# gudovskiy/contextflow

Measured on AMD Instinct MI355X. Metric: samples/s fwd+logdet (log p(x) (B,M)), CIFAR-10C conv flow, higher is better.
Workload: dtype f32

## Files before the change

contextflow_amd/csrc/cf_step.hip:

```cpp
#include "cf_step_common.h"
#include "cf_step_inv.h"
#include "cf_step_dispatch.h"

namespace {

struct StepArgs {
    const float* x;
    float* z;
    float* ldj;
    const float* ws;
    int B;
    int64_t xbs;
    bool sq;
    hipStream_t s;
    float* dbg = nullptr;
    const float* sb = nullptr;
    StepTape tp = kNoTape;
};

constexpr int kPrepBatch = 16;
struct StepPackBatch {
    const float *Wm[kPrepBatch], *t[kPrepBatch], *logs[kPrepBatch], *w1[kPrepBatch], *b1[kPrepBatch], *w2[kPrepBatch], *b2[kPrepBatch],
        *w3[kPrepBatch], *b3[kPrepBatch];
    float* ws[kPrepBatch];
// ... 138 lines not shown
constexpr int kChain = 4;
struct WsChain { const float* ws[kChain]; };

template <class G, int CTX, bool DUMP, bool DBG, bool LEVEL>
__device__ __forceinline__ void flow_step_phases(float* __restrict__ z, float* __restrict__ ldj_acc, const float* __restrict__ wsl, int B,
                                                 float* __restrict__ dbg_arg, const float* __restrict__ sb, StepTape tp, int tile, int wave_u = 0) {
    float* const dbg = DBG ? dbg_arg : nullptr;
    constexpr int C = G::C, HW = G::HW, PIX = G::PIX, HALF = G::HALF, HID = G::HID;
    constexpr int PTW = G::PTW, RT03 = G::RT03;
    constexpr int WPX = 32 * PTW;
    static_assert(!LEVEL || (CTX == 0 && !DUMP && !DBG && HW <= 32 * PTW), "level form: the evaluation step, log-det inside the wave");
    extern __shared__ __align__(16) float lds[];
    float* Y0 = lds;
    float* H1 = lds + HALF * PIX;

    const int tid_ = LEVEL ? wave_u * 64 + cf_lane_fresh() : (int)threadIdx.x;
    const int tid = tid_, wave = tid >> 6;
    int lane = tid & 63, li = lane & 31, lk = lane >> 5;
    const int ntiles = (B + G::SPW - 1) / G::SPW;
    const int64_t dbg_cols = (int64_t)ntiles * PIX;

    int pix[PTW], pin[PTW];
#pragma unroll
    for (int q = 0; q < PTW; ++q) {
        pix[q] = (wave * PTW + q) * 32 + li;
        pin[q] = pix[q] % HW;
    }
    {
        const int b0 = tile * G::SPW;
        int smp[PTW];
        bool live[PTW];
// ... 16 lines not shown
                const int idx = tile_row(r, lk);
                if (idx < HALF) Y0[idx * PIX + pix[q]] = acc0[0][q][r];
                y1[q][r] = (HALF <= 16) ? acc0[0][q][r + 8] : acc0[RT03 - 1][q][r];
            }
        if constexpr (LEVEL) {
#pragma unroll
            for (int q = 0; q < PTW; ++q)
#pragma unroll
                for (int r = 0; r < (HALF <= 16 ? 8 : 16); ++r) asm volatile("" : "+v"(y1[q][r]));
        }
        cf_wave_sync();
        if constexpr (!LEVEL) z_store<G>(z, Y0, b0, 0, B, wave, lane);
        if constexpr (DUMP) rows_store_t<G, HALF, HALF>(tp.y0, Y0, b0, B, wave, lane);
        if (dbg) {
            __syncthreads();
            for (int e = tid; e < HALF * PIX; e += 256) dbg[(int64_t)(e / PIX) * dbg_cols + (int64_t)tile * PIX + (e % PIX)] = Y0[e];
            __syncthreads();
        }

        f32x16 acc3[RT03][PTW];
        if constexpr (LEVEL) {
            conditioner_net<G, 0, false, 2>(acc3, lds, wsl, pix, pin, lane, tid, nullptr, 0, tile, nullptr, nullptr, tp, B);
            lane = cf_lane_fresh(); li = lane & 31; lk = lane >> 5;
#pragma unroll
            for (int q = 0; q < PTW; ++q) {
                pix[q] = (wave_u * PTW + q) * 32 + li;
                pin[q] = pix[q] % HW;
                smp[q] = b0 + pix[q] / HW;
                live[q] = smp[q] < B;
            }
#pragma unroll
            for (int rt = 0; rt < RT03; ++rt)
#pragma unroll
                for (int q = 0; q < PTW; ++q) acc3[rt][q] = bias_tile(wsl + G::OFF_B3 + rt * 32, lk);
            dense_phase<G, G::KS3, G::NG3, RT03>(acc3, ws_rsrc(wsl, G::WS_FLOATS), G::OFF_A3, H1, pix, lane);
        } else if constexpr (CTX == 0) {
            conditioner_net<G, 0, DUMP>(acc3, lds, wsl, pix, pin, lane, tid, dbg, dbg_cols, tile, nullptr, nullptr, tp, B);
        } else {
// ... 70 lines not shown
            if (tid < G::SPW && b0 + tid < B) {
                float sum = 0.f;
#pragma unroll
                for (int i = 0; i < TPS; ++i) {
                    const int t = tid * TPS + i;
                    sum += Y0[(t / PTW) * WPX + (t % PTW)];
                }
                ldj_acc[b0 + tid] += wsl[0] + sum;
            }
            __syncthreads();
        }
    }
}

template <class G, bool SQ, int CTX = 0, bool DUMP = false, bool DBG = false>
__global__ __launch_bounds__(256, G::MINW) void k_flow_step(const float* __restrict__ x, float* __restrict__ z,
                                                   float* __restrict__ ldj_acc, const float* __restrict__ ws, int B,
                                                   int64_t xbs, float* __restrict__ dbg_arg, int flags,
                                                   const float* __restrict__ sb, StepTape tp) {
    constexpr int XI = G::C * G::PTW / 8;
    extern __shared__ __align__(16) float lds[];
    float* H1 = lds + G::HALF * G::PIX;
    const int tid = threadIdx.x, lane = tid & 63, wave = tid >> 6;
    (void)flags;

    float4 xr[XI];
    const int tile = blockIdx.x;
    x_load<G, SQ>(xr, x, xbs, tile, B, wave, lane);
    x_to_lds<G, SQ>(xr, H1, wave, lane);
    flow_step_phases<G, CTX, DUMP, DBG, false>(z, ldj_acc, ws, B, dbg_arg, sb, tp, tile);
}
template <class G, bool SQ>
__global__ __launch_bounds__(256, G::MINW) void k_flow_step_level(const float* __restrict__ x, float* __restrict__ z,
                                                                  float* __restrict__ ldj_acc, const WsChain wc, int nsteps, int B, int64_t xbs) {
    constexpr int XI = G::C * G::PTW / 8;
    extern __shared__ __align__(16) float lds[];
    float* H1 = lds + G::HALF * G::PIX;
    const int tid = threadIdx.x, lane = tid & 63, wave = tid >> 6;
    const int tile = blockIdx.x, wave_u = __builtin_amdgcn_readfirstlane(wave);
    {
        float4 xr[XI];
        x_load<G, SQ>(xr, x, xbs, tile, B, wave, lane);
        x_to_lds<G, SQ>(xr, H1, wave, lane);
    }
#pragma unroll 1
// ... 763 lines not shown
    if (rc) return rc;
    int blocks = (G::WS_FLOATS + 255) / 256;
    if (blocks > 512) blocks = 512;
    k_step_pack<G><<<dim3(blocks, n), dim3(256), 0, s>>>(pb);
    return 0;
}

template <class G, bool SQ, int CTX, bool DUMP, bool DBG>
int launch_step_sq(const StepArgs& a) {
    constexpr size_t lds_bytes = (size_t)G::LDS_FLOATS * sizeof(float);
    if (lds_bytes > 64 * 1024) {
        static std::atomic<uint64_t> raised{0};
        if (int rc_ = cf_raise_dynamic_lds((const void*)k_flow_step<G, SQ, CTX, DUMP, DBG>, 160 * 1024, raised, __func__)) return rc_;
    }
    const int grid = (a.B + G::SPW - 1) / G::SPW;
    k_flow_step<G, SQ, CTX, DUMP, DBG><<<dim3(grid), dim3(256), lds_bytes, a.s>>>(a.x, a.z, a.ldj, a.ws, a.B, a.xbs, a.dbg, 0, a.sb, a.tp);
    return 0;
}
template <class G, int CTX = 0, bool DUMP = false, bool DBG = false>
int launch_step(const StepArgs& a) {
    if constexpr (CTX == 0) { if (a.sq) return launch_step_sq<G, true, CTX, DUMP, DBG>(a); }
    return launch_step_sq<G, false, CTX, DUMP, DBG>(a);
}

template <class G, bool SQ>
int launch_step_level_sq(const StepArgs& a, const WsChain& wc, int n) {
    constexpr size_t lds_bytes = (size_t)G::LDS_FLOATS * sizeof(float);
    if (lds_bytes > 64 * 1024) {
        static std::atomic<uint64_t> raised{0};
        if (int rc_ = cf_raise_dynamic_lds((const void*)k_flow_step_level<G, SQ>, 160 * 1024, raised, __func__)) return rc_;
    }
// ... 14 lines not shown
        case Kernel::None: return 0;
        case Kernel::Small_G8s: return step_macs_c2hw<G8s>();
        case Kernel::Small_G16s: return step_macs_c2hw<G16s>();
        case Kernel::Small_G8w: case Kernel::Inv_G8w: return step_macs_c2hw<G8w>();
        case Kernel::Small_G16w: case Kernel::Inv_G16w: return step_macs_c2hw<G16w>();
        case Kernel::Step_G8: case Kernel::Inv_G8: return step_macs_c2hw<G8>();
        case Kernel::Step_G16: case Kernel::Inv_G16: return step_macs_c2hw<G16>();
        case Kernel::Step_G32: case Kernel::Rs_G32: case Kernel::Inv_G32: return step_macs_c2hw<G32>();
        case Kernel::Step_G32v2: return step_macs_c2hw<G32v2>();
        case Kernel::Step_G32w: case Kernel::Inv_G32w: return step_macs_c2hw<G32w>();
        case Kernel::Step_G32w24: return step_macs_c2hw<G32w24>();
        case Kernel::Step_G64: case Kernel::Rs16_G64: case Kernel::Inv_G64: return step_macs_c2hw<G64>();
        case Kernel::Step_G64v2: return step_macs_c2hw<G64v2>();
        case Kernel::Step_G64w2: case Kernel::Inv_G64w2: return step_macs_c2hw<G64w2>();
        case Kernel::Step_G64w24: return step_macs_c2hw<G64w24>();
    }
    return 0;
}

static int launch_fwd(Kernel k, const StepArgs& a) {
    switch (k) {
        case Kernel::Small_G8s: return launch_step_small<G8s>(a);
        case Kernel::Small_G16s: return launch_step_small<G16s>(a);
        case Kernel::Small_G8w: return launch_step_small<G8w>(a);
        case Kernel::Small_G16w: return launch_step_small<G16w>(a);
        case Kernel::Step_G8: return launch_step<G8>(a);
        case Kernel::Step_G16: return launch_step<G16>(a);
        case Kernel::Step_G32: return launch_step<G32>(a);
        case Kernel::Step_G32v2: return launch_step<G32v2>(a);
        case Kernel::Step_G32w: return launch_step<G32w>(a);
        case Kernel::Step_G32w24: return launch_step<G32w24>(a);
        case Kernel::Step_G64: return launch_step<G64>(a);
        case Kernel::Step_G64v2: return launch_step<G64v2>(a);
        case Kernel::Step_G64w2: return launch_step<G64w2>(a);
        case Kernel::Step_G64w24: return launch_step<G64w24>(a);
        case Kernel::Rs_G32: return launch_step_rs<G32, 2>(a);
        case Kernel::Rs16_G64: return launch_step_rs16<G64>(a);
        default: return not_built(__func__, k);
    }
}
static int launch_fwd_dumps(Kernel k, const StepArgs& a) {
    switch (k) {
        case Kernel::Small_G8s: return launch_step_small<G8s, true>(a);
        case Kernel::Small_G16s: return launch_step_small<G16s, true>(a);
        case Kernel::Step_G8: return launch_step<G8, 0, false, true>(a);
        case Kernel::Step_G16: return launch_step<G16, 0, false, true>(a);
        case Kernel::Step_G32: return launch_step<G32, 0, false, true>(a);
        case Kernel::Step_G64: return launch_step<G64, 0, false, true>(a);
        default: return not_built(__func__, k);
    }
// ... 82 lines not shown

template <class G>
static int lane_table_copy(int* out, int cap) {
    static const LaneTab<G> tab = make_lane_tab<G>();
    constexpr int n = (int)(sizeof(LaneEntry<G>) / sizeof(int));
    static_assert(sizeof(tab) == 256 * n * sizeof(int), "an entry is n ints, no padding");
    const int* src = reinterpret_cast<const int*>(&tab);
    for (int i = 0; out && i < cap && i < 256 * n; ++i) out[i] = src[i];
    return n;
}
constexpr int kDebugVariants = 8;
constexpr Kernel kDebugKernel[4][kDebugVariants] = {
    {Kernel::Step_G8, Kernel::None, Kernel::None, Kernel::Small_G8s, Kernel::Small_G8w, Kernel::None, Kernel::None, Kernel::None},
    {Kernel::Step_G16, Kernel::None, Kernel::None, Kernel::Small_G16s, Kernel::Small_G16w, Kernel::None, Kernel::None, Kernel::None},
    {Kernel::Step_G32, Kernel::None, Kernel::Step_G32v2, Kernel::None, Kernel::Step_G32w, Kernel::None, Kernel::Step_G32w24, Kernel::None},
    {Kernel::Step_G64, Kernel::None, Kernel::Step_G64v2, Kernel::None, Kernel::None, Kernel::Step_G64w2, Kernel::Step_G64w24, Kernel::None},
};

extern "C" {

int cf_flow_step_supported(int C, int H, int W, int kh, int kw) {
    return (kh == 3 && kw == 3 && shape_id(C, H, W) >= 0) ? 1 : 0;
}

int64_t cf_flow_step_ws_bytes(int C, int H, int W) {
    switch (shape_id(C, H, W)) {
        case 0: return (int64_t)G8::WS_FLOATS * 4;
        case 1: return (int64_t)G16::WS_FLOATS * 4;
        case 2: return (int64_t)G32::WS_FLOATS * 4;
        case 3: return (int64_t)G64::WS_FLOATS * 4;
    }
// ... 129 lines not shown
    if (B == 0) return 0;
    CF_REQUIRE(x && z && ldj_acc && ws && B >= 0 && x_bstride >= (int64_t)C * H * W);
    CF_REQUIRE((reinterpret_cast<uintptr_t>(x) & 15) == 0 && (reinterpret_cast<uintptr_t>(z) & 15) == 0 && x_bstride % 4 == 0);
    const int sid = shape_id(C, H, W), variant = (flags >> 16) & 15;
    const Kernel k = (sid >= 0 && variant < kDebugVariants) ? kDebugKernel[sid][variant] : Kernel::None;
    if (k == Kernel::None) {
        cf_set_error("cf_flow_step_fwd: shape (%d,%d,%d) variant %d unsupported", C, H, W, variant);
        return CF_ERR_UNSUPPORTED;
    }
    StepArgs a{x, z, ldj_acc, (const float*)ws, B, x_bstride, in_squeeze != 0, cf_s(stream)};
    a.dbg = dbg;
    if (int rc = dbg ? launch_fwd_dumps(k, a) : launch_fwd(k, a)) return rc;
    CF_LAUNCH_CHECK();
    return 0;
}
int cf_lane_table_debug(int C, int H, int W, int* out, int cap) {
    switch (shape_id(C, H, W)) {
        case 1: static_assert(kLaneTabW22<G16w>, "16x16, C = 16: F(2x2) table"); return lane_table_copy<G16w>(out, cap);
        case 2: static_assert(kLaneTabW24<G32w24>, "8x8: F(2x4) table"); return lane_table_copy<G32w24>(out, cap);    }
    return 0;
}
int cf_flow_step_chain_max_batch(int C, int H, int W) { return chain_max_batch(shape_id(C, H, W)); }

int cf_flow_step_fwd_chain(const float* x, float* z, float* ldj_acc, const void* const* ws, int n, int B, int C, int H, int W,
                           int64_t x_bstride, int in_squeeze, cf_stream_t stream) {
    if (B == 0 || n == 0) return 0;
    CF_REQUIRE(x && z && ldj_acc && ws && n >= 1 && n <= kChain && B > 0 && x_bstride >= (int64_t)C * H * W);
    CF_REQUIRE((reinterpret_cast<uintptr_t>(x) & 15) == 0 && (reinterpret_cast<uintptr_t>(z) & 15) == 0 && x_bstride % 4 == 0);
    const Kernel k = select(Pass::Chain, shape_id(C, H, W), B);
    if (k == Kernel::None) {
// ... 8 lines not shown
}

int cf_flow_step_level_min_batch(int C, int H, int W) { return level_min_batch(shape_id(C, H, W)); }

int cf_flow_step_fwd_level(const float* x, float* z, float* ldj_acc, const void* const* ws, int n, int B, int C, int H, int W,
                           int64_t x_bstride, int in_squeeze, int form, cf_stream_t stream) {
    if (B == 0 || n == 0) return 0;
    CF_REQUIRE(x && z && x != z && ldj_acc && ws && n >= 1 && n <= kChain && B > 0 && x_bstride >= (int64_t)C * H * W && (form == 0 || form == 1));
    CF_REQUIRE((reinterpret_cast<uintptr_t>(x) & 15) == 0 && (reinterpret_cast<uintptr_t>(z) & 15) == 0 && x_bstride % 4 == 0);
    const int sid = shape_id(C, H, W), minb = level_min_batch(sid);
    if (sid < 0) return unsupported_shape(__func__, C, H, W);
    if (minb == 0 || (form == 0 && B < minb)) {
        cf_set_error("cf_flow_step_fwd_level: shape (%d,%d,%d) at a batch of %d is not a level case", C, H, W, B);
        return CF_ERR_UNSUPPORTED;
    }
    const Kernel k = select(Pass::Eval, sid, form == 1 && B < minb ? minb : B);
    WsChain wc{};
    for (int i = 0; i < n; ++i) { CF_REQUIRE(ws[i]); wc.ws[i] = (const float*)ws[i]; }
    if (int rc = launch_fwd_level(k, StepArgs{x, z, ldj_acc, nullptr, B, x_bstride, in_squeeze != 0, cf_s(stream)}, wc, n)) return rc;
    CF_LAUNCH_CHECK();
    return 0;
}

int cf_flow_step_fwd(const float* x, float* z, float* ldj_acc, const void* ws, int B, int C, int H, int W,
                     int64_t x_bstride, int in_squeeze, cf_stream_t stream) {
    if (B == 0) return 0;
    CF_REQUIRE(x && z && ldj_acc && ws && B >= 0 && x_bstride >= (int64_t)C * H * W);
    CF_REQUIRE((reinterpret_cast<uintptr_t>(x) & 15) == 0 && (reinterpret_cast<uintptr_t>(z) & 15) == 0 && x_bstride % 4 == 0);
    const Kernel k = select(Pass::Eval, shape_id(C, H, W), B);
    if (k == Kernel::None) return unsupported_shape(__func__, C, H, W);
    if (int rc = launch_fwd(k, StepArgs{x, z, ldj_acc, (const float*)ws, B, x_bstride, in_squeeze != 0, cf_s(stream)})) return rc;
// ... 68 lines not shown
```

contextflow_amd/csrc/cf_step_common.h:

```cpp
#pragma once
#include <type_traits>
#include "cf_common.h"
#include <math.h>

namespace {


typedef float f32x16 __attribute__((ext_vector_type(16)));

constexpr int kWaves = 4;

template <int C_, int H_, int W_, int SPW_, int PIPE_ = 1, int ABL_ = 0, int PATCH_ = 0>
struct Geo {
    static constexpr int C = C_, H = H_, W = W_, SPW = SPW_, PIPE = PIPE_, ABL = ABL_, PATCH = PATCH_;
    static constexpr int HW = H * W;
    static constexpr int PIX = SPW * HW;
    static constexpr int HALF = C / 2;
    static constexpr int HID = 2 * C;
    static constexpr int NPT = PIX / 32;
    static constexpr int PTW = NPT / kWaves;
    static constexpr int HP = HALF <= 16 ? 16 : 32;
    static constexpr int R03 = 2 * HP;
    static constexpr int RT03 = R03 / 32;
    static constexpr int RT1 = (HID + 31) / 32;
    static constexpr int R1 = RT1 * 32;
    static constexpr int KS0 = C / 2, KS1 = HALF / 2, KS3 = HID / 2;
    static constexpr int NG0 = (KS0 + 3) / 4, NG1 = (KS1 + 3) / 4, NG3 = (KS3 + 3) / 4;
    static constexpr int NCG = HID / 8;
    static constexpr int NG2 = 9 * NCG;
    static constexpr int OFF_B0 = 4, OFF_B1 = OFF_B0 + R03, OFF_B2 = OFF_B1 + R1, OFF_B3 = OFF_B2 + R1;
    static constexpr int OFF_A0 = OFF_B3 + R03;
    static constexpr int OFF_A1 = OFF_A0 + NG0 * RT03 * 256;
    static constexpr int OFF_A2 = OFF_A1 + NG1 * RT1 * 256;
    static constexpr int OFF_A3 = OFF_A2 + NG2 * RT1 * 256;
    static constexpr bool SMALL = (H == 16 && W == 16 && SPW == 1 && C <= 16);
// ... 14 lines not shown
    static constexpr int OFF_RA0 = OFF_RB3 + C, OFF_RA1 = OFF_RA0 + (C / 16) * (C / 16) * 256;
    static constexpr int OFF_RA2 = OFF_RA1 + (HID / 16) * (HALF / 16) * 256, OFF_RA3 = OFF_RA2 + (HID / 16) * 9 * (HID / 16) * 256;
    static constexpr int R16_END = OFF_RA3 + (C / 16) * (HID / 16) * 256;
    static constexpr int WS_END0 = RS16 ? R16_END : OFF_AW + 16 * HID * HID;
    static constexpr bool HAS_W24 = (H == 4 && W == 4) || (H == 8 && W == 8);
    static constexpr int OFF_AW24 = WS_END0;
    static constexpr int WS_FLOATS = OFF_AW24 + (HAS_W24 ? 24 * HID * HID : 0);
    static constexpr int PP = 2 * W + 2 * H + 4;
    static constexpr int RS = PATCH ? ((PIX + SPW * PP + 1 + 3) & ~3) : PIX;
#ifndef CF_WINO_LDSW
#define CF_WINO_LDSW 1
#endif
    static constexpr int LDS_W = (CF_WINO_LDSW && PIPE_ == 3 && HID == 16 && H == 16 && W == 16 && SPW == 1) ? 16 * HID * HID : 0;
    static constexpr int LDS_FLOATS = (HALF + HID) * RS + LDS_W;
    static constexpr int MINW = (160 * 1024) / (LDS_FLOATS * 4) >= 4 ? 4 : ((160 * 1024) / (LDS_FLOATS * 4) >= 2 ? 2 : 1);
    static_assert(PIX % 128 == 0 && PTW >= 1, "workgroup must own a multiple of 128 pixels");
    static_assert(!W24 || (H == 4 && W == 4 && SPW == 8) || (H == 8 && W == 8 && SPW == 4),
                  "F(2x4, 3x3): 4x4 images, 8 samples = one column tile of 16 output tiles; 8x8 images, 4 samples = two column tiles");
    static_assert(HID % 8 == 0 && C % 4 == 0, "channel counts must fill whole k-steps");
    static_assert((HW & (HW - 1)) == 0 && (W & (W - 1)) == 0, "power-of-two images");
};

template <class G> constexpr bool kLaneTabW24 = G::W24 && G::H == 8;
template <class G> constexpr bool kLaneTabW22 = G::PIPE == 3 && G::SMALL && G::C == 16;

template <class G> __host__ __device__ constexpr int chan_of_row(int p) {
    return ((p % G::HP) < G::HALF) ? (p / G::HP) * G::HALF + (p % G::HP) : -1;
}

template <class G> __host__ __device__ constexpr int chan_of_row16(int p) {
    return (2 * (p >> 2) + (p & 1) < G::HALF) ? ((p & 2) ? G::HALF : 0) + 2 * (p >> 2) + (p & 1) : -1;
}

// ... 586 lines not shown
#pragma unroll
            for (int i = 0; i < 2; ++i) {
                float* dst = kLaneTabW22<G> ? H1 + (rt0 + rt) * 16 * PIX + i * W + dsto
                                            : H1 + ((rt0 + rt) * 16 + 4 * lg) * PIX + smp[ct] * HW + (2 * ty[ct] + i) * W + 2 * tx[ct];
                const float bb[4] = {b.x, b.y, b.z, b.w};
#pragma unroll
                for (int r = 0; r < 4; ++r)
                    *reinterpret_cast<float2*>(dst + r * PIX) =
                        make_float2(cf_relu(Y[ct][i][0][rt][r] + bb[r]), cf_relu(Y[ct][i][1][rt][r] + bb[r]));
            }
    }
    if constexpr (RSPLIT > 1) __syncthreads();
    else cf_wave_sync();
}

template <class G> __host__ __device__ constexpr int w24_row(int s, int y, int kq) {
    return 128 * (s >> 1) + 32 * ((y ^ (kq >> 1)) & 1) + 8 * (y >> 1) + 4 * (s & 1);
}
template <class G> __host__ __device__ constexpr int w24_col(int x, int kq) {
    return 64 * ((x >> 1) & 1) + 2 * (((x >> 2) ^ (x >> 1)) & 1) + ((x ^ kq) & 1);
}
template <class G> __host__ __device__ constexpr int w24_pix(int s, int y, int x, int kq) {
    if constexpr (G::H == 4) return 8 * (4 * y + ((x + y + kq) & 3)) + s;
    else return w24_row<G>(s, y, kq) + w24_col<G>(x, kq);
}

constexpr int cf_reflect(int v, int n) { return v < 0 ? -v : (v >= n ? 2 * (n - 1) - v : v); }
template <class G> struct alignas(16) W24Lane {
    int row[4];
    int col[6];
    int dst;
    int pad;
    int pw[G::PTW][4];
};
template <class G> __host__ __device__ constexpr W24Lane<G> w24_lane(int wave, int lane) {
    static_assert(kLaneTabW24<G>, "tabulated for the 8x8 level");
    constexpr int W = G::W, H = G::H, HW = G::HW, PIX = G::PIX, HALF = G::HALF, NCT = PIX / 128, TPS = HW / 8, TXN = W / 4;
    W24Lane<G> e{};
// ... 23 lines not shown
    const int l15 = lane & 15, lg = lane >> 4, li = lane & 31;
    const int tg = wave * 16 + l15, ti = tg % TPS;
    const int smp = tg / TPS, ty = ti / (W / 2), tx = ti % (W / 2);
    for (int a = 0; a < 4; ++a) {
        const int yy = cf_reflect(2 * ty - 1 + a, H), xx = cf_reflect(2 * tx - 1 + a, W);
        e.row[a] = 4 * (HALF * PIX + lg * PIX + wino_pix<G>(smp * HW, yy, 0));
        e.col[a] = 4 * ((((xx ^ lg) & 1) * (W / 2)) + (xx >> 1));
    }
    for (int q = 0; q < 2; ++q) {
        const int pix = (wave * G::PTW + q) * 32 + li, pin = pix % HW;
        e.pw[q] = wino_pix<G>(pix - pin, pin / W, pin % W);
    }
    e.dst = 4 * lg * PIX + smp * HW + 2 * ty * W + 2 * tx;
    return e;
}
template <class G> using LaneEntry = std::conditional_t<G::W24, W24Lane<G>, W22Lane<G>>;
template <class G> struct LaneTab { LaneEntry<G> e[kWaves * 64]; };
template <class G> constexpr LaneTab<G> make_lane_tab() {
    LaneTab<G> t{};
    for (int i = 0; i < kWaves * 64; ++i) {
        if constexpr (G::W24) t.e[i] = w24_lane<G>(i >> 6, i & 63);
        else t.e[i] = w22_lane<G>(i >> 6, i & 63);
    }
    return t;
}
template <class G> __device__ const LaneTab<G> kLaneTab = make_lane_tab<G>();
template <class G> __device__ __forceinline__ int4 lane_tab_word(int tid, int i) {
    return reinterpret_cast<const int4*>(&kLaneTab<G>.e[tid])[i];
}

#ifndef CF_W24_SPREAD
#define CF_W24_SPREAD 1
#endif
template <class G>
__device__ __forceinline__ void winograd24_phase2(float* __restrict__ lds, const float* __restrict__ wsl, ws_rsrc_t rs, int lane,
                                                  int wave, const int4 (&tw)[3]) {
    constexpr int W = G::W, H = G::H, HW = G::HW, PIX = G::PIX, HALF = G::HALF, RT16 = G::RT16, KG4 = G::KG4;
    constexpr int NCT = PIX / 128;
    constexpr int RSP = kWaves / NCT;
    static_assert(G::W24 && (NCT == 1 || NCT == 2) && RT16 % RSP == 0 && W % 4 == 0, "F(2x4, 3x3) geometry");
    constexpr int RTW = RT16 / RSP;
    constexpr int NS = 6 * KG4;
    constexpr int NU[6] = {0, 5, 1, 2, 3, 4};
    typedef float f32x2w __attribute__((ext_vector_type(2)));
    constexpr bool SPREAD = CF_W24_SPREAD && H == 8;
    const int rt0 = __builtin_amdgcn_readfirstlane((NCT == 1 ? wave : wave / NCT) * RTW);
    float* H1 = lds + HALF * PIX;
    const int l15 = lane & 15, lg = lane >> 4;
    const int smp = l15 >> 1, ty = l15 & 1;
    int yrow[4];
    int rpart[4], cpart[6], dsto = 0;
    if constexpr (H == 4) {
#pragma unroll
        for (int a = 0; a < 4; ++a) {
            const int yy = 2 * ty - 1 + a;
            yrow[a] = yy < 0 ? -yy : (yy >= H ? 2 * (H - 1) - yy : yy);
        }
    } else {
        const int4 t0 = tw[0], t1 = tw[1], t2 = tw[2];
        rpart[0] = t0.x; rpart[1] = t0.y; rpart[2] = t0.z; rpart[3] = t0.w;
        cpart[0] = t1.x; cpart[1] = t1.y; cpart[2] = t1.z; cpart[3] = t1.w; cpart[4] = t2.x; cpart[5] = t2.y;
        dsto = t2.z;
    }
    f32x4w Y[2][4][RTW];
#pragma unroll
    for (int i = 0; i < 2; ++i)
#pragma unroll
        for (int j = 0; j < 4; ++j)
#pragma unroll
            for (int rt = 0; rt < RTW; ++rt) Y[i][j][rt] = f32x4w{0.f, 0.f, 0.f, 0.f};
    auto addrs = [&](int xi, int (&o)[2][6]) {
#pragma unroll
        for (int h = 0; h < 2; ++h) {
            if constexpr (H == 4) {
                const int yy = h == 0 ? (xi == 0 ? yrow[0] : (xi == 2 ? yrow[2] : yrow[1]))
                                      : (xi == 2 ? yrow[1] : (xi == 3 ? yrow[3] : yrow[2]));
#pragma unroll
                for (int c = 0; c < 6; ++c) {
                    const int xx = c == 0 ? 1 : (c == 5 ? 2 : c - 1);
                    o[h][c] = 4 * (HALF * PIX + lg * PIX + w24_pix<G>(smp, yy, xx, lg & 1));
                }
            } else {
                const int rr = h == 0 ? (xi == 0 ? rpart[0] : (xi == 2 ? rpart[2] : rpart[1]))
                                      : (xi == 2 ? rpart[1] : (xi == 3 ? rpart[3] : rpart[2]));
#pragma unroll
                for (int c = 0; c < 6; ++c) o[h][c] = rr + cpart[c];
            }
        }
    };
// ... 7 lines not shown
#pragma unroll
                for (int e2 = 0; e2 < 2; ++e2) {
                    const char* q0 = reinterpret_cast<const char*>(lds) + (16 * kk + 8 * e2) * PIX * 4;
                    const char* q1 = q0 + 4 * PIX * 4;
                    r.d[h][c][e2] = f32x2w{*reinterpret_cast<const float*>(q0 + o[h][c]), *reinterpret_cast<const float*>(q1 + o[h][c])};
                }
    };
    auto load_raw = [&](const int (&o)[2][6], int kk, Raw& r) { load_raw_cols(o, kk, r, 0, 6); };
    auto load_w = [&](int xi, int s, WFrag& f) {
        const int kk = s / 6, nu = NU[s % 6];
        const int fr = G::OFF_AW24 + (((xi * 6 + nu) * RT16 + rt0) * KG4 + kk) * 256;
#pragma unroll
        for (int rt = 0; rt < RTW; ++rt) f.a[rt] = ws_frag(rs, lane, fr + rt * KG4 * 256);
    };
    int o[2][6];
    addrs(0, o);
    Raw raw;
    WFrag wf[2];
    load_raw(o, 0, raw);
    load_w(0, 0, wf[0]);
    auto xi_body = [&](const int xi, auto has0, auto has1) {
        const int xn = xi < 3 ? xi + 1 : 3;
        const float sigma = xi == 1 ? 1.f : -1.f;
        const float c0 = xi < 3 ? 1.f : 0.f, c1 = xi == 0 ? 0.f : (xi == 1 ? 1.f : -1.f);
        f32x4w M[6][RTW];
#pragma unroll
        for (int nu = 0; nu < 6; ++nu)
#pragma unroll
            for (int rt = 0; rt < RTW; ++rt) M[nu][rt] = f32x4w{0.f, 0.f, 0.f, 0.f};
#pragma unroll
        for (int kk = 0; kk < KG4; ++kk) {
            f32x2w A[6][2];
#pragma unroll
            for (int c = 0; c < 6; ++c)
#pragma unroll
                for (int e2 = 0; e2 < 2; ++e2) A[c][e2] = raw.d[0][c][e2] + sigma * raw.d[1][c][e2];
            if (kk + 1 == KG4) addrs(xn, o);
            const int kn = kk + 1 < KG4 ? kk + 1 : 0;
            if constexpr (!SPREAD) load_raw(o, kn, raw);
            auto operand = [&](const int nu, f32x2w (&v)[2]) {
#pragma unroll
                for (int e2 = 0; e2 < 2; ++e2) {
                    const f32x2w a0 = A[0][e2], a1 = A[1][e2], a2 = A[2][e2], a3 = A[3][e2], a4 = A[4][e2], a5 = A[5][e2];
                    if (nu == 0) v[e2] = 0.25f * a0 + (a4 - 1.25f * a2);
                    else if (nu == 1) v[e2] = (a4 - 0.25f * a2) + (a3 - 0.25f * a1);
                    else if (nu == 2) v[e2] = (a4 - 0.25f * a2) - (a3 - 0.25f * a1);
                    else if (nu == 3) v[e2] = (a4 - a2) + 0.5f * (a3 - a1);
                    else if (nu == 4) v[e2] = (a4 - a2) - 0.5f * (a3 - a1);
                    else v[e2] = 0.25f * a1 + (a5 - 1.25f * a3);
                }
            };
#pragma unroll
            for (int t = 0; t < 6; ++t) {
                const int s = kk * 6 + t, nu = NU[t];
                if (s + 1 < NS) load_w(xi, s + 1, wf[(s + 1) & 1]);
                else load_w(xn, 0, wf[0]);
                if constexpr (SPREAD) load_raw_cols(o, kn, raw, t, t + 1);
                __builtin_amdgcn_sched_barrier(0);
                f32x2w v[2];
                operand(nu, v);
                const WFrag& f = wf[s & 1];
#pragma unroll
                for (int e = 0; e < 4; ++e)
#pragma unroll
                    for (int rt = 0; rt < RTW; ++rt)
                        M[nu][rt] = __builtin_amdgcn_mfma_f32_16x16x4f32(f4e(f.a[rt], e), v[e >> 1][e & 1], M[nu][rt], 0, 0, 0);
                __builtin_amdgcn_sched_barrier(0);
            }
        }
#pragma unroll
        for (int rt = 0; rt < RTW; ++rt) {
            const f32x4w s12 = M[1][rt] + M[2][rt], d12 = M[1][rt] - M[2][rt], s34 = M[3][rt] + M[4][rt], d34 = M[3][rt] - M[4][rt];
            const f32x4w Z[4] = {M[0][rt] + s12 + s34, d12 + 0.5f * d34, s12 + 0.25f * s34, d12 + 0.125f * d34 + M[5][rt]};
#pragma unroll
            for (int j = 0; j < 4; ++j) {
                if constexpr (decltype(has0)::value) Y[0][j][rt] += c0 * Z[j];
                if constexpr (decltype(has1)::value) Y[1][j][rt] += c1 * Z[j];
            }
        }
    };
    xi_body(0, std::true_type{}, std::false_type{});
#pragma unroll 1
    for (int xi = 1; xi < 3; ++xi) xi_body(xi, std::true_type{}, std::true_type{});
    xi_body(3, std::false_type{}, std::true_type{});
    __syncthreads();
#pragma unroll
    for (int rt = 0; rt < RTW; ++rt) {
        const float4 b = *reinterpret_cast<const float4*>(wsl + G::OFF_B2 + (rt0 + rt) * 16 + 4 * lg);
        const float bb[4] = {b.x, b.y, b.z, b.w};
#pragma unroll
        for (int i = 0; i < 2; ++i)
#pragma unroll
            for (int r = 0; r < 4; ++r) {
                float* dst = H == 4 ? H1 + ((rt0 + rt) * 16 + 4 * lg + r) * PIX + smp * HW + (2 * ty + i) * W
                                    : H1 + ((rt0 + rt) * 16 + r) * PIX + i * W + dsto;
                *reinterpret_cast<float4*>(dst) = make_float4(cf_relu(Y[i][0][rt][r] + bb[r]), cf_relu(Y[i][1][rt][r] + bb[r]),
                                                              cf_relu(Y[i][2][rt][r] + bb[r]), cf_relu(Y[i][3][rt][r] + bb[r]));
            }
    }
// ... 77 lines not shown
                            const int row = rt * 32 + tile_row(r, lk);
                            if (row < HID) dst[row * G::HW] = cf_relu(acc[rt][q][r]);
                        }
                }
            }
            mask_store<G, RT1>(tp.m1, acc, tile, tid >> 6, lane);
        } else if constexpr (DUMP) {
            cf_wave_sync();
            rows_store_t<G, HID, HID>(tp.h1, H1, tile * G::SPW, B, tid >> 6, lane);
            mask_store<G, RT1>(tp.m1, acc, tile, tid >> 6, lane);
        }
    }
    __syncthreads();
    if (dbg) {
        float* d = dbg + (int64_t)C * dbg_cols;
        for (int e = tid; e < HID * PIX; e += 256) d[(int64_t)(e / PIX) * dbg_cols + (int64_t)tile * PIX + (e % PIX)] = H1[e];
    }

    if constexpr (G::WINO) {
        if constexpr (G::W24) {
            static_assert(!DUMP, "the F(2x4) form runs in the evaluation forward only");
            winograd24_phase2<G>(lds, wsl, rs, lane, tid >> 6, tw2);
        } else {
            winograd_phase2<G>(lds, wsl, rs, lane, tid >> 6, tw2);
        }
        if constexpr (DUMP) {
            rows_store_t<G, HID, HID>(tp.h2, H1, tile * G::SPW, B, tid >> 6, lane);
#pragma unroll
            for (int rt = 0; rt < RT1; ++rt)
#pragma unroll
                for (int q = 0; q < PTW; ++q) {
// ... 139 lines not shown
            for (int q = 0; q < PTW; ++q)
#pragma unroll
                for (int r = 0; r < 16; ++r) {
                    const int row = rt * 32 + tile_row(r, lk);
                    if (row < HID) H1[row * PIX + pix[q]] = cf_relu(acc[rt][q][r]);
                }
        cf_wave_sync();
        if constexpr (DUMP) {
            rows_store_t<G, HID, HID>(tp.h2, H1, tile * G::SPW, B, tid >> 6, lane);
            mask_store<G, RT1>(tp.m2, acc, tile, tid >> 6, lane);
        }
    }
    if (dbg) {
        __syncthreads();
        float* d = dbg + (int64_t)(C + HID) * dbg_cols;
        for (int e = tid; e < HID * PIX; e += 256) d[(int64_t)(e / PIX) * dbg_cols + (int64_t)tile * PIX + (e % PIX)] = H1[e];
    }

    if constexpr (UPTO < 3) return;
#pragma unroll
    for (int rt = 0; rt < RT03; ++rt)
#pragma unroll
        for (int q = 0; q < PTW; ++q) acc3[rt][q] = bias_tile(wsl + G::OFF_B3 + rt * 32, lk);
    if constexpr (CTX == 1) {
#pragma unroll
        for (int rt = 0; rt < RT03; ++rt)
#pragma unroll
            for (int q = 0; q < PTW; ++q)
#pragma unroll
                for (int r = 0; r < 16; ++r) {
                    const int ch = chan_of_row<G>(rt * 32 + (r & 3) + 8 * (r >> 2)) ;
// ... 7 lines not shown

using G8 = Geo<8, 16, 16, 1, 0>;
using G16 = Geo<16, 16, 16, 1, 0>;
using G32 = Geo<32, 8, 8, 4, 1>;
using G64 = Geo<64, 4, 4, 16, 1>;
using G16s = Geo<16, 16, 16, 1, 2>;
using G8s = Geo<8, 16, 16, 1, 2>;
using G32v2 = Geo<32, 8, 8, 2, 1>;
using G64v2 = Geo<64, 4, 4, 8, 1>;
using G8w = Geo<8, 16, 16, 1, 3>;
using G16w = Geo<16, 16, 16, 1, 3>;
using G32w = Geo<32, 8, 8, 4, 3>;
using G64w2 = Geo<64, 4, 4, 8, 3>;
using G64w24 = Geo<64, 4, 4, 8, 6>;
using G32w24 = Geo<32, 8, 8, 4, 6>;


int shape_id(int C, int H, int W) {
    if (C == 8 && H == 16 && W == 16) return 0;
    if (C == 16 && H == 16 && W == 16) return 1;
    if (C == 32 && H == 8 && W == 8) return 2;
    if (C == 64 && H == 4 && W == 4) return 3;
    return -1;
}

}
```

contextflow_amd/csrc/cf_step_dispatch.h:

```cpp
#pragma once
#include "cf_step_common.h"
#include <cstdlib>

static bool direct_conv_only() {
    static const bool v = [] { const char* e = getenv("CONTEXTFLOW_DIRECT_CONV"); return e && e[0] == '1'; }();
    return v;
}
enum class Kernel {
    None,
    Small_G8s, Small_G16s, Small_G8w, Small_G16w,
    Step_G8, Step_G16, Step_G32, Step_G32v2, Step_G32w, Step_G32w24, Step_G64, Step_G64v2, Step_G64w2, Step_G64w24,
    Rs_G32,
    Rs16_G64,
    Inv_G8, Inv_G8w, Inv_G16, Inv_G16w, Inv_G32, Inv_G32w, Inv_G64, Inv_G64w2,
};
enum class Pass { Eval, Taped, Ctx, CtxDirect, CtxTaped, Chain, Inverse, InverseCtx };

constexpr int kFullMinB8x8 = 256 * G32::SPW;
constexpr int kFullMinB4x4 = 256 * G64::SPW;
constexpr int kWinoMinB4x4 = 256 * G64w2::SPW;
constexpr int kW24MinB8x8 = 512 * G32w24::SPW;
constexpr int kRsMaxB8x8 = 512;
constexpr int kRs16MaxB4x4 = 1024;
constexpr int kChainMaxB16x16 = 1024;

static int chain_max_batch(int sid) {
    switch (sid) {
        case 0: case 1: return direct_conv_only() ? 0 : kChainMaxB16x16;
        case 2: return kRsMaxB8x8;
        case 3: return kRs16MaxB4x4;
    }
    return 0;
}

static Kernel select(Pass pass, int sid, int B) {
    const bool direct = direct_conv_only() || pass == Pass::CtxDirect;
    const bool eval = pass == Pass::Eval, ctx = pass == Pass::Ctx || pass == Pass::CtxDirect;
    if (pass == Pass::Inverse || pass == Pass::InverseCtx) {
        const bool ictx = pass == Pass::InverseCtx;
        const bool d = direct && !ictx;
        switch (sid) {
            case 0: return d || ictx ? Kernel::Inv_G8 : Kernel::Inv_G8w;
            case 1: return d ? Kernel::Inv_G16 : Kernel::Inv_G16w;
            case 2: return d ? Kernel::Inv_G32 : Kernel::Inv_G32w;
            case 3: return d ? Kernel::Inv_G64 : Kernel::Inv_G64w2;
            default: return Kernel::None;
        }
    }
    if (pass == Pass::CtxTaped)
        switch (sid) {
            case 0: return Kernel::Step_G8;
            case 1: return Kernel::Step_G16;
// ... 5 lines not shown
    switch (sid) {
        case 0:
            if (ctx) return Kernel::Step_G8;
            return (pass != Pass::Taped && !direct) ? Kernel::Small_G8w : Kernel::Small_G8s;
        case 1:
            if (direct) return ctx ? Kernel::Step_G16 : Kernel::Small_G16s;
            return Kernel::Small_G16w;
        case 2:
            if (!ctx && B <= kRsMaxB8x8) return Kernel::Rs_G32;
            if (B < kFullMinB8x8) return ctx ? Kernel::Step_G32 : Kernel::Step_G32v2;
            if (direct) return Kernel::Step_G32;
            if (eval && B >= kW24MinB8x8) return Kernel::Step_G32w24;
            return Kernel::Step_G32w;
        case 3:
            if (!ctx && B <= kRs16MaxB4x4) return Kernel::Rs16_G64;
            if (!direct && B >= kWinoMinB4x4) return eval ? Kernel::Step_G64w24 : Kernel::Step_G64w2;
            return (!ctx && B < kFullMinB4x4) ? Kernel::Step_G64v2 : Kernel::Step_G64;
    }
    return Kernel::None;
}

static int not_built(const char* fn, Kernel k) {
    cf_set_error("%s: kernel %d is not built for this pass", fn, (int)k);
    return CF_ERR_UNSUPPORTED;
}
static int unsupported_shape(const char* fn, int C, int H, int W) {
    cf_set_error("%s: shape (%d,%d,%d) unsupported", fn, C, H, W);
    return CF_ERR_UNSUPPORTED;
}
```

Measured before the change: 3.915 million.

## Add zero-skip F(2x4) Winograd variant for 4x4 level on 8 waves

Adds a new G64z24 geometry for the 4x4, C=64 level that handles 16 samples per workgroup on 8 waves. Each wave owns one output tile row, and for each row it skips the Winograd input-transform column whose two patch rows collapse to the same image row under reflect padding, so that term is exactly zero. This removes redundant loads and MFMA work in the 3x3 conv and changes the pixel lane layout and the block size. It is selected only for eval passes at very large batch (65536 and above) and can be toggled at runtime, at the cost of higher register and LDS pressure per workgroup.

New measurement: 4.030 million (median of 6 runs). 1.03x the previous value.

```diff
diff --git a/contextflow_amd/csrc/cf_step.hip b/contextflow_amd/csrc/cf_step.hip
--- a/contextflow_amd/csrc/cf_step.hip
+++ b/contextflow_amd/csrc/cf_step.hip
@@ -176,7 +176,9 @@
     float* Y0 = lds;
     float* H1 = lds + HALF * PIX;
 
-    const int tid_ = LEVEL ? wave_u * 64 + cf_lane_fresh() : (int)threadIdx.x;
+    constexpr bool FRESH = LEVEL || G::ZSKIP;
+    static_assert(!G::ZSKIP || (CTX == 0 && !DUMP && !DBG), "zero skip: the evaluation step");
+    const int tid_ = FRESH ? wave_u * 64 + cf_lane_fresh() : (int)threadIdx.x;
     const int tid = tid_, wave = tid >> 6;
     int lane = tid & 63, li = lane & 31, lk = lane >> 5;
     const int ntiles = (B + G::SPW - 1) / G::SPW;
@@ -223,14 +225,15 @@
         if constexpr (DUMP) rows_store_t<G, HALF, HALF>(tp.y0, Y0, b0, B, wave, lane);
         if (dbg) {
             __syncthreads();
-            for (int e = tid; e < HALF * PIX; e += 256) dbg[(int64_t)(e / PIX) * dbg_cols + (int64_t)tile * PIX + (e % PIX)] = Y0[e];
+            for (int e = tid; e < HALF * PIX; e += G::NT) dbg[(int64_t)(e / PIX) * dbg_cols + (int64_t)tile * PIX + (e % PIX)] = Y0[e];
             __syncthreads();
         }
 
         f32x16 acc3[RT03][PTW];
-        if constexpr (LEVEL) {
+        if constexpr (FRESH) {
             conditioner_net<G, 0, false, 2>(acc3, lds, wsl, pix, pin, lane, tid, nullptr, 0, tile, nullptr, nullptr, tp, B);
             lane = cf_lane_fresh(); li = lane & 31; lk = lane >> 5;
+            if constexpr (G::ZSKIP) lk &= 1;
 #pragma unroll
             for (int q = 0; q < PTW; ++q) {
                 pix[q] = (wave_u * PTW + q) * 32 + li;
@@ -331,7 +334,7 @@
 }
 
 template <class G, bool SQ, int CTX = 0, bool DUMP = false, bool DBG = false>
-__global__ __launch_bounds__(256, G::MINW) void k_flow_step(const float* __restrict__ x, float* __restrict__ z,
+__global__ __launch_bounds__(G::NT, G::MINW) void k_flow_step(const float* __restrict__ x, float* __restrict__ z,
                                                    float* __restrict__ ldj_acc, const float* __restrict__ ws, int B,
                                                    int64_t xbs, float* __restrict__ dbg_arg, int flags,
                                                    const float* __restrict__ sb, StepTape tp) {
@@ -345,7 +348,8 @@
     const int tile = blockIdx.x;
     x_load<G, SQ>(xr, x, xbs, tile, B, wave, lane);
     x_to_lds<G, SQ>(xr, H1, wave, lane);
-    flow_step_phases<G, CTX, DUMP, DBG, false>(z, ldj_acc, ws, B, dbg_arg, sb, tp, tile);
+    if constexpr (G::ZSKIP) flow_step_phases<G, CTX, DUMP, DBG, false>(z, ldj_acc, ws, B, dbg_arg, sb, tp, tile, __builtin_amdgcn_readfirstlane(wave));
+    else flow_step_phases<G, CTX, DUMP, DBG, false>(z, ldj_acc, ws, B, dbg_arg, sb, tp, tile);
 }
 template <class G, bool SQ>
 __global__ __launch_bounds__(256, G::MINW) void k_flow_step_level(const float* __restrict__ x, float* __restrict__ z,
@@ -1139,7 +1143,7 @@
         if (int rc_ = cf_raise_dynamic_lds((const void*)k_flow_step<G, SQ, CTX, DUMP, DBG>, 160 * 1024, raised, __func__)) return rc_;
     }
     const int grid = (a.B + G::SPW - 1) / G::SPW;
-    k_flow_step<G, SQ, CTX, DUMP, DBG><<<dim3(grid), dim3(256), lds_bytes, a.s>>>(a.x, a.z, a.ldj, a.ws, a.B, a.xbs, a.dbg, 0, a.sb, a.tp);
+    k_flow_step<G, SQ, CTX, DUMP, DBG><<<dim3(grid), dim3(G::NT), lds_bytes, a.s>>>(a.x, a.z, a.ldj, a.ws, a.B, a.xbs, a.dbg, 0, a.sb, a.tp);
     return 0;
 }
 template <class G, int CTX = 0, bool DUMP = false, bool DBG = false>
@@ -1184,6 +1188,7 @@
         case Kernel::Step_G64v2: return step_macs_c2hw<G64v2>();
         case Kernel::Step_G64w2: case Kernel::Inv_G64w2: return step_macs_c2hw<G64w2>();
         case Kernel::Step_G64w24: return step_macs_c2hw<G64w24>();
+        case Kernel::Step_G64z24: return step_macs_c2hw<G64z24>();
     }
     return 0;
 }
@@ -1204,6 +1209,7 @@
         case Kernel::Step_G64v2: return launch_step<G64v2>(a);
         case Kernel::Step_G64w2: return launch_step<G64w2>(a);
         case Kernel::Step_G64w24: return launch_step<G64w24>(a);
+        case Kernel::Step_G64z24: return launch_step<G64z24>(a);
         case Kernel::Rs_G32: return launch_step_rs<G32, 2>(a);
         case Kernel::Rs16_G64: return launch_step_rs16<G64>(a);
         default: return not_built(__func__, k);
@@ -1316,7 +1322,7 @@
     {Kernel::Step_G8, Kernel::None, Kernel::None, Kernel::Small_G8s, Kernel::Small_G8w, Kernel::None, Kernel::None, Kernel::None},
     {Kernel::Step_G16, Kernel::None, Kernel::None, Kernel::Small_G16s, Kernel::Small_G16w, Kernel::None, Kernel::None, Kernel::None},
     {Kernel::Step_G32, Kernel::None, Kernel::Step_G32v2, Kernel::None, Kernel::Step_G32w, Kernel::None, Kernel::Step_G32w24, Kernel::None},
-    {Kernel::Step_G64, Kernel::None, Kernel::Step_G64v2, Kernel::None, Kernel::None, Kernel::Step_G64w2, Kernel::Step_G64w24, Kernel::None},
+    {Kernel::Step_G64, Kernel::None, Kernel::Step_G64v2, Kernel::None, Kernel::None, Kernel::Step_G64w2, Kernel::Step_G64w24, Kernel::Step_G64z24},
 };
 
 extern "C" {
@@ -1476,6 +1482,10 @@
     CF_LAUNCH_CHECK();
     return 0;
 }
+int cf_flow_step_zero_skip_min_batch(int C, int H, int W) {
+    return select(Pass::Eval, shape_id(C, H, W), kZeroSkipMinB4x4) == Kernel::Step_G64z24 ? kZeroSkipMinB4x4 : 0;
+}
+int cf_flow_step_zero_skip_enable(int on) { return g_zero_skip.exchange(on != 0) ? 1 : 0; }
 int cf_lane_table_debug(int C, int H, int W, int* out, int cap) {
     switch (shape_id(C, H, W)) {
         case 1: static_assert(kLaneTabW22<G16w>, "16x16, C = 16: F(2x2) table"); return lane_table_copy<G16w>(out, cap);
@@ -1514,7 +1524,7 @@
         cf_set_error("cf_flow_step_fwd_level: shape (%d,%d,%d) at a batch of %d is not a level case", C, H, W, B);
         return CF_ERR_UNSUPPORTED;
     }
-    const Kernel k = select(Pass::Eval, sid, form == 1 && B < minb ? minb : B);
+    const Kernel k = select(Pass::Level, sid, form == 1 && B < minb ? minb : B);
     WsChain wc{};
     for (int i = 0; i < n; ++i) { CF_REQUIRE(ws[i]); wc.ws[i] = (const float*)ws[i]; }
     if (int rc = launch_fwd_level(k, StepArgs{x, z, ldj_acc, nullptr, B, x_bstride, in_squeeze != 0, cf_s(stream)}, wc, n)) return rc;
diff --git a/contextflow_amd/csrc/cf_step_common.h b/contextflow_amd/csrc/cf_step_common.h
--- a/contextflow_amd/csrc/cf_step_common.h
+++ b/contextflow_amd/csrc/cf_step_common.h
@@ -13,12 +13,14 @@
 template <int C_, int H_, int W_, int SPW_, int PIPE_ = 1, int ABL_ = 0, int PATCH_ = 0>
 struct Geo {
     static constexpr int C = C_, H = H_, W = W_, SPW = SPW_, PIPE = PIPE_, ABL = ABL_, PATCH = PATCH_;
+    static constexpr bool ZSKIP = PIPE_ == 6 && H_ == 4 && SPW_ == 16;
+    static constexpr int WAVES = ZSKIP ? 8 : kWaves, NT = 64 * WAVES;
     static constexpr int HW = H * W;
     static constexpr int PIX = SPW * HW;
     static constexpr int HALF = C / 2;
     static constexpr int HID = 2 * C;
     static constexpr int NPT = PIX / 32;
-    static constexpr int PTW = NPT / kWaves;
+    static constexpr int PTW = NPT / WAVES;
     static constexpr int HP = HALF <= 16 ? 16 : 32;
     static constexpr int R03 = 2 * HP;
     static constexpr int RT03 = R03 / 32;
@@ -63,9 +65,10 @@
     static constexpr int LDS_W = (CF_WINO_LDSW && PIPE_ == 3 && HID == 16 && H == 16 && W == 16 && SPW == 1) ? 16 * HID * HID : 0;
     static constexpr int LDS_FLOATS = (HALF + HID) * RS + LDS_W;
     static constexpr int MINW = (160 * 1024) / (LDS_FLOATS * 4) >= 4 ? 4 : ((160 * 1024) / (LDS_FLOATS * 4) >= 2 ? 2 : 1);
-    static_assert(PIX % 128 == 0 && PTW >= 1, "workgroup must own a multiple of 128 pixels");
-    static_assert(!W24 || (H == 4 && W == 4 && SPW == 8) || (H == 8 && W == 8 && SPW == 4),
+    static_assert(PIX % 128 == 0 && PTW >= 1 && NPT % WAVES == 0, "workgroup must own a multiple of 128 pixels");
+    static_assert(!W24 || (H == 4 && W == 4 && SPW == 8) || (H == 8 && W == 8 && SPW == 4) || ZSKIP,
                   "F(2x4, 3x3): 4x4 images, 8 samples = one column tile of 16 output tiles; 8x8 images, 4 samples = two column tiles");
+    static_assert(!ZSKIP || (W == 4 && WAVES == 8 && C == 64), "zero skip: 16 samples of the 4x4 level on 8 waves, the whole LDS");
     static_assert(HID % 8 == 0 && C % 4 == 0, "channel counts must fill whole k-steps");
     static_assert((HW & (HW - 1)) == 0 && (W & (W - 1)) == 0, "power-of-two images");
 };
@@ -682,6 +685,10 @@
     else cf_wave_sync();
 }
 
+__host__ __device__ constexpr int w24z_pix(int s, int y, int x, int kq) {
+    const int R = 2 * y + (x >> 1);
+    return 32 * R + 16 * ((x ^ kq) & 1) + ((s ^ (2 * R)) & 15);
+}
 template <class G> __host__ __device__ constexpr int w24_row(int s, int y, int kq) {
     return 128 * (s >> 1) + 32 * ((y ^ (kq >> 1)) & 1) + 8 * (y >> 1) + 4 * (s & 1);
 }
@@ -689,7 +696,8 @@
     return 64 * ((x >> 1) & 1) + 2 * (((x >> 2) ^ (x >> 1)) & 1) + ((x ^ kq) & 1);
 }
 template <class G> __host__ __device__ constexpr int w24_pix(int s, int y, int x, int kq) {
-    if constexpr (G::H == 4) return 8 * (4 * y + ((x + y + kq) & 3)) + s;
+    if constexpr (G::ZSKIP) return w24z_pix(s, y, x, kq);
+    else if constexpr (G::H == 4) return 8 * (4 * y + ((x + y + kq) & 3)) + s;
     else return w24_row<G>(s, y, kq) + w24_col<G>(x, kq);
 }
 
@@ -743,6 +751,11 @@
     e.dst = 4 * lg * PIX + smp * HW + 2 * ty * W + 2 * tx;
     return e;
 }
+constexpr int w24_r1(int xi) { return xi == 0 ? 0 : (xi == 2 ? 2 : 1); }
+constexpr int w24_r2(int xi) { return xi == 2 ? 1 : (xi == 3 ? 3 : 2); }
+constexpr bool w24_xi_is_zero(int xi, int ty, int H) {
+    return xi != 1 && cf_reflect(2 * ty - 1 + w24_r1(xi), H) == cf_reflect(2 * ty - 1 + w24_r2(xi), H);
+}
 template <class G> using LaneEntry = std::conditional_t<G::W24, W24Lane<G>, W22Lane<G>>;
 template <class G> struct LaneTab { LaneEntry<G> e[kWaves * 64]; };
 template <class G> constexpr LaneTab<G> make_lane_tab() {
@@ -766,8 +779,11 @@
                                                   int wave, const int4 (&tw)[3]) {
     constexpr int W = G::W, H = G::H, HW = G::HW, PIX = G::PIX, HALF = G::HALF, RT16 = G::RT16, KG4 = G::KG4;
     constexpr int NCT = PIX / 128;
-    constexpr int RSP = kWaves / NCT;
+    constexpr int RSP = G::WAVES / NCT;
     static_assert(G::W24 && (NCT == 1 || NCT == 2) && RT16 % RSP == 0 && W % 4 == 0, "F(2x4, 3x3) geometry");
+    constexpr bool ZS = G::ZSKIP;
+    static_assert(!ZS || (NCT == 2 && HW / 8 == 2 && w24_xi_is_zero(0, 0, H) && w24_xi_is_zero(3, 1, H)),
+                  "zero skip: the two patch rows of the skipped (xi, ty) must be ONE image row under the padding, and be subtracted");
     constexpr int RTW = RT16 / RSP;
     constexpr int NS = 6 * KG4;
     constexpr int NU[6] = {0, 5, 1, 2, 3, 4};
@@ -776,7 +792,8 @@
     const int rt0 = __builtin_amdgcn_readfirstlane((NCT == 1 ? wave : wave / NCT) * RTW);
     float* H1 = lds + HALF * PIX;
     const int l15 = lane & 15, lg = lane >> 4;
-    const int smp = l15 >> 1, ty = l15 & 1;
+    const int ct = ZS ? __builtin_amdgcn_readfirstlane(wave % NCT) : 0;
+    const int smp = ZS ? l15 : l15 >> 1, ty = ZS ? ct : l15 & 1;
     int yrow[4];
     int rpart[4], cpart[6], dsto = 0;
     if constexpr (H == 4) {
@@ -793,7 +810,7 @@
     }
     f32x4w Y[2][4][RTW];
 #pragma unroll
-    for (int i = 0; i < 2; ++i)
+    for (int i = 0; i < (ZS ? 1 : 2); ++i)
 #pragma unroll
         for (int j = 0; j < 4; ++j)
 #pragma unroll
@@ -802,6 +819,8 @@
 #pragma unroll
         for (int h = 0; h < 2; ++h) {
             if constexpr (H == 4) {
+                static_assert(w24_r1(0) == 0 && w24_r1(1) == 1 && w24_r1(2) == 2 && w24_r1(3) == 1 && w24_r2(0) == 2 && w24_r2(1) == 2 &&
+                              w24_r2(2) == 1 && w24_r2(3) == 3, "the rows below are w24_r1 / w24_r2, which the zero-skip check reads");
                 const int yy = h == 0 ? (xi == 0 ? yrow[0] : (xi == 2 ? yrow[2] : yrow[1]))
                                       : (xi == 2 ? yrow[1] : (xi == 3 ? yrow[3] : yrow[2]));
 #pragma unroll
@@ -839,12 +858,15 @@
         for (int rt = 0; rt < RTW; ++rt) f.a[rt] = ws_frag(rs, lane, fr + rt * KG4 * 256);
     };
     int o[2][6];
-    addrs(0, o);
+    int hoff = (KG4 / 2) * 16 * PIX * 4;
+    if constexpr (ZS) asm volatile("" : "+s"(hoff));
+    const int xi_first = ZS && ct == 0 ? 1 : 0;
+    addrs(xi_first, o);
     Raw raw;
     WFrag wf[2];
     load_raw(o, 0, raw);
-    load_w(0, 0, wf[0]);
-    auto xi_body = [&](const int xi, auto has0, auto has1) {
+    load_w(xi_first, 0, wf[0]);
+    auto xi_body = [&](const int xi, auto has0, auto has1, const bool stop) {
         const int xn = xi < 3 ? xi + 1 : 3;
         const float sigma = xi == 1 ? 1.f : -1.f;
         const float c0 = xi < 3 ? 1.f : 0.f, c1 = xi == 0 ? 0.f : (xi == 1 ? 1.f : -1.f);
@@ -862,7 +884,15 @@
                 for (int e2 = 0; e2 < 2; ++e2) A[c][e2] = raw.d[0][c][e2] + sigma * raw.d[1][c][e2];
             if (kk + 1 == KG4) addrs(xn, o);
             const int kn = kk + 1 < KG4 ? kk + 1 : 0;
-            if constexpr (!SPREAD) load_raw(o, kn, raw);
+            if constexpr (ZS) {
+                if (kk + 1 == KG4 / 2) {
+#pragma unroll
+                    for (int h = 0; h < 2; ++h)
+#pragma unroll
+                        for (int c = 0; c < 6; ++c) o[h][c] += hoff;
+                }
+                if (kk + 1 < KG4 || !stop) load_raw(o, kn % (KG4 / 2), raw);
+            } else if constexpr (!SPREAD) load_raw(o, kn, raw);
             auto operand = [&](const int nu, f32x2w (&v)[2]) {
 #pragma unroll
                 for (int e2 = 0; e2 < 2; ++e2) {
@@ -879,7 +909,7 @@
             for (int t = 0; t < 6; ++t) {
                 const int s = kk * 6 + t, nu = NU[t];
                 if (s + 1 < NS) load_w(xi, s + 1, wf[(s + 1) & 1]);
-                else load_w(xn, 0, wf[0]);
+                else if (!ZS || !stop) load_w(xn, 0, wf[0]);
                 if constexpr (SPREAD) load_raw_cols(o, kn, raw, t, t + 1);
                 __builtin_amdgcn_sched_barrier(0);
                 f32x2w v[2];
@@ -904,10 +934,16 @@
             }
         }
     };
-    xi_body(0, std::true_type{}, std::false_type{});
+    if (!ZS || ct == 1) xi_body(0, std::true_type{}, std::false_type{}, false);
+    if constexpr (ZS) {
+#pragma unroll
+        for (int j = 0; j < 4; ++j)
+#pragma unroll
+            for (int rt = 0; rt < RTW; ++rt) Y[1][j][rt] = f32x4w{0.f, 0.f, 0.f, 0.f};
+    }
 #pragma unroll 1
-    for (int xi = 1; xi < 3; ++xi) xi_body(xi, std::true_type{}, std::true_type{});
-    xi_body(3, std::false_type{}, std::true_type{});
+    for (int xi = 1; xi < 3; ++xi) xi_body(xi, std::true_type{}, std::true_type{}, ZS && ct == 1 && xi == 2);
+    if (!ZS || ct == 0) xi_body(3, std::false_type{}, std::true_type{}, true);
     __syncthreads();
 #pragma unroll
     for (int rt = 0; rt < RTW; ++rt) {
@@ -1015,7 +1051,7 @@
     __syncthreads();
     if (dbg) {
         float* d = dbg + (int64_t)C * dbg_cols;
-        for (int e = tid; e < HID * PIX; e += 256) d[(int64_t)(e / PIX) * dbg_cols + (int64_t)tile * PIX + (e % PIX)] = H1[e];
+        for (int e = tid; e < HID * PIX; e += G::NT) d[(int64_t)(e / PIX) * dbg_cols + (int64_t)tile * PIX + (e % PIX)] = H1[e];
     }
 
     if constexpr (G::WINO) {
@@ -1185,7 +1221,7 @@
     if (dbg) {
         __syncthreads();
         float* d = dbg + (int64_t)(C + HID) * dbg_cols;
-        for (int e = tid; e < HID * PIX; e += 256) d[(int64_t)(e / PIX) * dbg_cols + (int64_t)tile * PIX + (e % PIX)] = H1[e];
+        for (int e = tid; e < HID * PIX; e += G::NT) d[(int64_t)(e / PIX) * dbg_cols + (int64_t)tile * PIX + (e % PIX)] = H1[e];
     }
 
     if constexpr (UPTO < 3) return;
@@ -1223,6 +1259,7 @@
 using G64w2 = Geo<64, 4, 4, 8, 3>;
 using G64w24 = Geo<64, 4, 4, 8, 6>;
 using G32w24 = Geo<32, 8, 8, 4, 6>;
+using G64z24 = Geo<64, 4, 4, 16, 6>;
 
 
 int shape_id(int C, int H, int W) {
diff --git a/contextflow_amd/csrc/cf_step_dispatch.h b/contextflow_amd/csrc/cf_step_dispatch.h
--- a/contextflow_amd/csrc/cf_step_dispatch.h
+++ b/contextflow_amd/csrc/cf_step_dispatch.h
@@ -1,5 +1,6 @@
 #pragma once
 #include "cf_step_common.h"
+#include <atomic>
 #include <cstdlib>
 
 static bool direct_conv_only() {
@@ -10,16 +11,20 @@
     None,
     Small_G8s, Small_G16s, Small_G8w, Small_G16w,
     Step_G8, Step_G16, Step_G32, Step_G32v2, Step_G32w, Step_G32w24, Step_G64, Step_G64v2, Step_G64w2, Step_G64w24,
+    Step_G64z24,
     Rs_G32,
     Rs16_G64,
     Inv_G8, Inv_G8w, Inv_G16, Inv_G16w, Inv_G32, Inv_G32w, Inv_G64, Inv_G64w2,
 };
-enum class Pass { Eval, Taped, Ctx, CtxDirect, CtxTaped, Chain, Inverse, InverseCtx };
+enum class Pass { Eval, Taped, Ctx, CtxDirect, CtxTaped, Chain, Inverse, InverseCtx, Level };
 
 constexpr int kFullMinB8x8 = 256 * G32::SPW;
 constexpr int kFullMinB4x4 = 256 * G64::SPW;
 constexpr int kWinoMinB4x4 = 256 * G64w2::SPW;
 constexpr int kW24MinB8x8 = 512 * G32w24::SPW;
+constexpr int kZeroSkipMinB4x4 = 65536;
+inline std::atomic<bool> g_zero_skip{true};
+static bool zero_skip_enabled() { return g_zero_skip.load(std::memory_order_relaxed); }
 constexpr int kRsMaxB8x8 = 512;
 constexpr int kRs16MaxB4x4 = 1024;
 constexpr int kChainMaxB16x16 = 1024;
@@ -35,7 +40,7 @@
 
 static Kernel select(Pass pass, int sid, int B) {
     const bool direct = direct_conv_only() || pass == Pass::CtxDirect;
-    const bool eval = pass == Pass::Eval, ctx = pass == Pass::Ctx || pass == Pass::CtxDirect;
+    const bool eval = pass == Pass::Eval || pass == Pass::Level, ctx = pass == Pass::Ctx || pass == Pass::CtxDirect;
     if (pass == Pass::Inverse || pass == Pass::InverseCtx) {
         const bool ictx = pass == Pass::InverseCtx;
         const bool d = direct && !ictx;
@@ -71,6 +76,7 @@
             return Kernel::Step_G32w;
         case 3:
             if (!ctx && B <= kRs16MaxB4x4) return Kernel::Rs16_G64;
+            if (!direct && pass == Pass::Eval && B >= kZeroSkipMinB4x4 && zero_skip_enabled()) return Kernel::Step_G64z24;
             if (!direct && B >= kWinoMinB4x4) return eval ? Kernel::Step_G64w24 : Kernel::Step_G64w2;
             return (!ctx && B < kFullMinB4x4) ? Kernel::Step_G64v2 : Kernel::Step_G64;
     }
```
